# vrettasm/VGPA

Measured on AMD Instinct MI355X. Metric: fwd+bwd sweeps/sec (free-energy+grad eval), Lorenz96 D=40 N=1000, higher is better.
Workload: dtype f64; 1 GPU; Lorenz96 D=40, RK4, Np=1001 (BASELINE configs[2]); batch_per_gpu=512, kernels=mfma

## Files before the change

### vgpa_amd/csrc/energy.hip

```cpp
#include "vgpa_internal.h"
#include "dispatch.h"
#include "energy_small.h"
#include "chol_wave.h"

namespace vgpa {
namespace {

constexpr int NT = 256;

__global__ void __launch_bounds__(NT) k_energy_1d(EnergyArgs a) {
  const int t = blockIdx.x * NT + threadIdx.x;
  const int prob = blockIdx.y;
  if (t >= a.Np) return;
  const size_t o = (size_t)prob * a.Np + t;
  const double la = a.A[(size_t)prob * a.strideA + t], ob = a.b[(size_t)prob * a.strideB + t], m = a.m[o], s = a.S[o];
  Energy1d r;
  const double th = a.theta_v ? a.theta_v[(size_t)prob * kMaxTheta] : a.theta[0];
  const double sg = a.sigma1_v ? a.sigma1_v[prob] : a.sigma1;
  if (a.model == VGPA_MODEL_OU) energy_1d<VGPA_MODEL_OU>(th, sg, la, ob, m, s, r);
  else energy_1d<VGPA_MODEL_DW>(th, sg, la, ob, m, s, r);
  if (a.hyp_only) { a.hyp[o] = r.hyp; return; }
  a.e_t[o] = r.e_t;
  a.Ef[o] = r.ef;
  if (a.Edf) a.Edf[o] = r.edf;
  a.dEm[o] = r.dm;
  a.dEs[o] = r.ds;
  if (a.hyp) a.hyp[o] = r.hyp;
}

__global__ void __launch_bounds__(64) k_energy_l63(EnergyArgs a) {
  const int t = blockIdx.x * 64 + threadIdx.x;
  const int prob = blockIdx.y;
  if (t >= a.Np) return;
  const size_t o = (size_t)prob * a.Np + t;
  const double* At = a.A + (size_t)prob * a.strideA + (size_t)t * 9;
  const double* bt = a.b + (size_t)prob * a.strideB + (size_t)t * 3;
  const double* mt = a.m + o * 3;
  const double* St = a.S + o * 9;
  double Av[9], bv[3], mv[3], Sv[9], isg[3];
  const double* th = a.theta_v ? a.theta_v + (size_t)prob * kMaxTheta : a.theta;
  const double* isgp = a.isg + (size_t)prob * a.isg_stride;
#pragma unroll
  for (int e = 0; e < 9; e++) { Av[e] = At[e]; Sv[e] = St[e]; }
#pragma unroll
  for (int i = 0; i < 3; i++) { bv[i] = bt[i]; mv[i] = mt[i]; isg[i] = isgp[i]; }
  EnergyL63 r;
  if (a.hyp) energy_l63<true>(th, isg, Av, bv, mv, Sv, r); else energy_l63<false>(th, isg, Av, bv, mv, Sv, r);
  if (a.hyp_only) {
    double* hp = a.hyp + o * 6;
#pragma unroll
    for (int i = 0; i < 6; i++) hp[i] = r.hyp[i];
    return;
  }
  a.e_t[o] = r.e_t;
  double* dm = a.dEm + o * 3;
  dm[0] = r.dm[0]; dm[1] = r.dm[1]; dm[2] = r.dm[2];
  double* ds = a.dEs + o * 9;
  ds[0] = r.ds[0]; ds[1] = r.ds[1]; ds[2] = r.ds[2];
  ds[3] = r.ds[1]; ds[4] = r.ds[3]; ds[5] = r.ds[4];
  ds[6] = r.ds[2]; ds[7] = r.ds[4]; ds[8] = r.ds[5];
  double* ef = a.Ef + o * 3;
  ef[0] = r.ef[0]; ef[1] = r.ef[1]; ef[2] = r.ef[2];
  if (a.hyp) {
    double* hp = a.hyp + o * 6;
#pragma unroll
    for (int i = 0; i < 6; i++) hp[i] = r.hyp[i];
  }
  if (a.Edf) {
    double* e = a.Edf + o * 9;
    const double vS = th[0], vR = th[1], vB = th[2];
    e[0] = -vS; e[1] = vS; e[2] = 0.0;
    e[3] = vR - mv[2]; e[4] = -1.0; e[5] = -mv[0];
    e[6] = mv[1]; e[7] = mv[0]; e[8] = -vB;
  }
}

__device__ __forceinline__ int wrap(int i, int n) { return i < 0 ? i + n : (i >= n ? i - n : i); }

__device__ __forceinline__ void wave_sync() {
  __builtin_amdgcn_fence(__ATOMIC_RELEASE, "wavefront");
  __builtin_amdgcn_wave_barrier();
  __builtin_amdgcn_fence(__ATOMIC_ACQUIRE, "wavefront");
}

__device__ __forceinline__ double lane_value(double v, int j) {
  const int lo = __builtin_amdgcn_readlane(__double2loint(v), j);
  const int hi = __builtin_amdgcn_readlane(__double2hiint(v), j);
  return __hiloint2double(hi, lo);
}

using cholw::chol_panel_pivots;
using cholw::rsqrt_pos;

__device__ __forceinline__ double wave_sum(double v) {
#pragma unroll
  for (int o = 32; o > 0; o >>= 1) v += __shfl_xor(v, o, 64);
  return v;
}

template <int NB>
struct WaveGemmGeo {
  static constexpr int NQ = NB / 4, REM = NB % 4, G = REM ? 4 / REM : 0;
  static constexpr int NLEFT = REM ? (NB + G - 1) / G : 0;
  static constexpr int NU = NB * NQ + NLEFT;
};

template <int NB, int MODE, int TRI = 0>
__device__ __forceinline__ void wave_gemm(const double* __restrict__ Aop, const double* __restrict__ Bm, int LD,
                                          double (&acc)[WaveGemmGeo<NB>::NU], const double* __restrict__ bscale = nullptr) {
  using g = WaveGemmGeo<NB>;
  const int l = threadIdx.x & 63, r4 = l >> 4, c4 = l & 3, b = (l >> 2) & 3;
  constexpr int rem = g::REM ? g::REM : 1;
#pragma unroll
  for (int u = 0; u < g::NU; u++) acc[u] = 0.0;
  const double* pa = Aop + r4 * LD + c4;
  const double* pb = Bm + r4 * LD;
  const int colq = l & 15;
  const int coll = 4 * (4 * g::NQ + b % rem) + c4;
  const int ileft = b / rem;
#pragma unroll
  for (int kk = 0; kk < NB; kk++) {
    const double bs = bscale ? bscale[4 * kk + r4] : 1.0;
    double bq[g::NQ > 0 ? g::NQ : 1];
#pragma unroll
    for (int q = 0; q < g::NQ; q++)
      if (kk >= 4 * q) bq[q] = bscale ? bs * pb[kk * 4 * LD + 16 * q + colq] : pb[kk * 4 * LD + 16 * q + colq];
    double bl = 0.0;
    if (g::NLEFT > 0 && kk >= 4 * g::NQ) bl = bscale ? bs * pb[kk * 4 * LD + coll] : pb[kk * 4 * LD + coll];
#pragma unroll
    for (int I = 0; I < NB; I++) {
      if (MODE == 1 && kk < I) continue;
      bool any = false;
#pragma unroll
      for (int q = 0; q < g::NQ; q++) any = any || (kk >= 4 * q && !(TRI == 1 && 4 * q + 3 < I) && !(TRI == 2 && 4 * q > I));
      if (!any) continue;
      const double af = pa[kk * 4 * LD + 4 * I];
#pragma unroll
      for (int q = 0; q < g::NQ; q++)
        if (kk >= 4 * q && !(TRI == 1 && 4 * q + 3 < I) && !(TRI == 2 && 4 * q > I)) acc[q * NB + I] = __builtin_amdgcn_mfma_f64_4x4x4f64(af, bq[q], acc[q * NB + I], 0, 0, 0);
    }
    if (g::NLEFT > 0 && kk >= 4 * g::NQ) {
#pragma unroll
      for (int v = 0; v < g::NLEFT; v++) {
        if (MODE == 1 && kk < v * g::G) continue;
        if (TRI == 2 && v * g::G + g::G - 1 < 4 * g::NQ) continue;
        int ib = v * g::G + ileft;
        ib = ib < NB ? ib : NB - 1;
        const double af = pa[kk * 4 * LD + 4 * ib];
        acc[NB * g::NQ + v] = __builtin_amdgcn_mfma_f64_4x4x4f64(af, bl, acc[NB * g::NQ + v], 0, 0, 0);
      }
    }
  }
}

template <int NB>
__device__ __forceinline__ void wave_gemm_elem(int u, int& row, int& col, bool& ok) {
  using g = WaveGemmGeo<NB>;
  const int l = threadIdx.x & 63, r4 = l >> 4, c4 = l & 3, b = (l >> 2) & 3;
  constexpr int rem = g::REM ? g::REM : 1;
  int Ib, Jb;
  if (u < NB * g::NQ) {
    const int q = u / NB;
    Ib = u - q * NB; Jb = 4 * q + b; ok = true;
  } else {
    const int v = u - NB * g::NQ;
    Ib = v * g::G + b / rem; Jb = 4 * g::NQ + b % rem;
    ok = (b < g::G * g::REM) && (Ib < NB);
  }
  row = 4 * Ib + r4; col = 4 * Jb + c4;
}

struct L96Lds {
  double *Lm, *Gm, *mv, *bv, *am, *sg, *vv, *dl, *qq, *rd;
};

__host__ __device__ inline int l96_dp(int D) { return 4 * ((D + 3) / 4); }
__host__ __device__ inline int l96_ld(int D) { return l96_dp(D) + 1; }
__host__ __device__ inline size_t l96_lds_doubles(int D) {
  return (size_t)2 * l96_dp(D) * l96_ld(D) + 7 * (size_t)l96_dp(D) + (2 * D + 1) + 8 + 4 * (size_t)l96_dp(D);
}

template <int NB>
__global__ void __launch_bounds__(64) k_energy_l96(EnergyArgs a) {
  extern __shared__ __attribute__((aligned(16))) double smem[];
  const int D = a.D, M = 2 * D + 1;
  constexpr int Dp = 4 * NB, LD = Dp + 1;
  const int l = threadIdx.x;
  const long long wid = blockIdx.x;
  const int prob = (int)(wid / a.Np), t = (int)(wid - (long long)prob * a.Np);
  const size_t o = (size_t)prob * a.Np + t;
  L96Lds S;
  S.Lm = smem; S.Gm = S.Lm + Dp * LD; S.mv = S.Gm + Dp * LD; S.bv = S.mv + Dp; S.am = S.bv + Dp; S.sg = S.am + Dp;
  S.dl = S.sg + Dp; S.qq = S.dl + Dp; S.rd = S.qq + Dp; S.vv = S.rd + Dp;
  const double* At = a.A + (size_t)prob * a.strideA + (size_t)t * D * D;
  const double* St = a.S + o * D * D;
  const double theta = a.theta_v ? lds_const(a.theta_v, prob * kMaxTheta) : a.theta[0];
  const double kappa = 1.05 * D, c = D + kappa;
  const bool act = l < D;
  const bool pad = l < Dp;
  const int li = pad ? l : Dp - 1;

  for (int e = l; e < Dp * LD; e += 64) { S.Lm[e] = 0.0; S.Gm[e] = 0.0; }
  if (pad) { S.mv[l] = 0.0; S.bv[l] = 0.0; S.sg[l] = 0.0; S.am[l] = 0.0; S.dl[l] = 0.0; S.qq[l] = 0.0; S.rd[l] = 1.0; }
  wave_sync();
  {
    constexpr int EPL = (Dp * Dp + 63) / 64;
    const int DD = D * D;
    const unsigned magic = ((1u << 20) + (unsigned)D - 1u) / (unsigned)D;
#pragma unroll
    for (int q0 = 0; q0 < EPL; q0 += 9) {
      double sv[9], av[9];
#pragma unroll
      for (int u = 0; u < 9; u++) {
        const int e = l + 64 * (q0 + u);
        const bool in = (q0 + u < EPL) && (e < DD);
        sv[u] = in ? St[e] : 0.0;
        av[u] = in ? At[e] : 0.0;
      }
#pragma unroll
      for (int u = 0; u < 9; u++) {
        const int e = l + 64 * (q0 + u);
        if ((q0 + u < EPL) && (e < DD)) {
          const int r = (int)(((unsigned)e * magic) >> 20), cc = e - r * D;
          S.Lm[r * LD + cc] = c * sv[u];
          S.Gm[cc * LD + r] = av[u];
        }
      }
    }
  }
  if (l >= D && pad) S.Lm[l * LD + l] = 1.0;
  if (act) { S.mv[l] = a.m[o * D + l]; S.bv[l] = a.b[(size_t)prob * a.strideB + (size_t)t * D + l]; S.sg[l] = a.isg[(size_t)prob * a.isg_stride + l]; }
  wave_sync();

  const int r4 = l >> 4, c4 = l & 3, b = (l >> 2) & 3;
  bool bad = false;
  double myrd = 1.0;
  const double* lrow_b = S.Lm + (4 * b + c4) * LD + r4;
  double* lout_b = S.Lm + (4 * b + r4) * LD + c4;
#pragma unroll
  for (int p = 0; p < NB; p++) {
    const int j0 = 4 * p;
    if (p > 0) {
      const double* brow = S.Lm + (j0 + c4) * LD + r4;
#pragma unroll
      for (int u = 0; p + 4 * u < NB; u++) {
        const bool full = p + 4 * u + 3 < NB;
        const bool rowok = full || (p + 4 * u + b < NB);
        const double* arow = full ? lrow_b + 4 * (p + 4 * u) * LD
                                  : S.Lm + (4 * (rowok ? p + 4 * u + b : NB - 1) + c4) * LD + r4;
        double uacc = 0.0;
#pragma unroll
        for (int kk = 0; kk < p; kk++) uacc = __builtin_amdgcn_mfma_f64_4x4x4f64(arow[4 * kk], brow[4 * kk], uacc, 0, 0, 0);
        if (rowok) lout_b[4 * (p + 4 * u) * LD + j0] -= uacc;
      }
      wave_sync();
    }
    chol_panel_pivots<LD>(S.Lm, myrd, j0, l, li, pad);
    wave_sync();
  }
  if (pad) S.rd[l] = myrd;
  wave_sync();
  bad = __any(!(myrd > 0.0 && myrd < __builtin_inf()));
  if (bad) {
    if (l == 0) atomicOr(a.status + prob, 1);
    return;
  }

  double* xdiag = S.vv + (2 * D + 1) + 7;
  if (l < NB) {
    const double* tb = S.Lm + (4 * l) * LD + 4 * l;
    const double x00 = S.rd[4 * l], x11 = S.rd[4 * l + 1], x22 = S.rd[4 * l + 2], x33 = S.rd[4 * l + 3];
    const double t10 = tb[LD], t20 = tb[2 * LD], t21 = tb[2 * LD + 1], t30 = tb[3 * LD], t31 = tb[3 * LD + 1], t32 = tb[3 * LD + 2];
    const double x10 = -(t10 * x00) * x11;
    const double x21 = -(t21 * x11) * x22;
    const double x32 = -(t32 * x22) * x33;
    const double x20 = -(t20 * x00 + t21 * x10) * x22;
    const double x31 = -(t31 * x11 + t32 * x21) * x33;
    const double x30 = -(t30 * x00 + t31 * x10 + t32 * x20) * x33;
    double* xo = xdiag + 16 * l;
    xo[0] = x00; xo[1] = 0.0; xo[2] = 0.0; xo[3] = 0.0;
    xo[4] = x10; xo[5] = x11; xo[6] = 0.0; xo[7] = 0.0;
    xo[8] = x20; xo[9] = x21; xo[10] = x22; xo[11] = 0.0;
    xo[12] = x30; xo[13] = x31; xo[14] = x32; xo[15] = x33;
  }
  {
    double s = 0.0;
#pragma unroll
    for (int k = 0; k < Dp; k++) s = __builtin_fma(S.Gm[k * LD + li], S.mv[k], s);
    if (act) { S.am[l] = s; if (a.Am) a.Am[o * D + l] = s; }
    double acc[WaveGemmGeo<NB>::NU];
    wave_gemm<NB, 0>(S.Gm, S.Lm, LD, acc);
    wave_sync();
#pragma unroll
    for (int u = 0; u < WaveGemmGeo<NB>::NU; u++) {
      int row, col; bool ok;
      wave_gemm_elem<NB>(u, row, col, ok);
      if (ok) S.Gm[row * LD + col] = acc[u];
    }
  }
  wave_sync();

  double vplus = 0.0, vminus = 0.0, v0 = 0.0, r0sq = 0.0;
  const bool hyper = a.hyp != nullptr;
  {
    auto col_of = [&](int q) { return q == 0 ? 0 : (q <= D ? q - 1 : q - 1 - D); };
    auto sgn_of = [&](int q) { return q == 0 ? 0.0 : (q <= D ? 1.0 : -1.0); };
    auto chi = [&](int q, int i) { return S.mv[i] + sgn_of(q) * S.Lm[i * LD + col_of(q)]; };
    const int jc = act ? l : 0;
    const int pP = 1 + jc, pM = 1 + D + jc;
    const int pPm = pP - 1, pPp = pP + 1;
    const int pMm = pM - 1, pMp = wrap(pM + 1, M);
    double am2 = chi(pPm, D - 2), am1 = chi(pPm, D - 1), a0 = chi(pP, 0), a1 = chi(pP, 1);
    double bm2 = chi(pMm, D - 2), bm1 = chi(pMm, D - 1), b0 = chi(pM, 0), b1 = chi(pM, 1);
    const double* lcol = S.Lm + jc;
    const double* gcol = S.Gm + jc;
#pragma unroll
    for (int i = 0; i < Dp; i++) {
      if (i >= D) break;
      const double gi = gcol[i * LD], ami = S.am[i], bvi = S.bv[i], sgi = S.sg[i];
      const double ra = ((a1 - am2) * am1 - a0 + theta) + (ami + gi) - bvi;
      const double rb = ((b1 - bm2) * bm1 - b0 + theta) + (ami - gi) - bvi;
      vplus = __builtin_fma(sgi, ra * ra, vplus);
      vminus = __builtin_fma(sgi, rb * rb, vminus);
      if (hyper && act) S.Gm[i * LD + jc] = ra * ra + rb * rb;
      am2 = am1; am1 = a0; a0 = a1;
      bm2 = bm1; bm1 = b0; b0 = b1;
      const int in = i + 2;
      if (in < D) {
        const double mi = S.mv[in], li2 = lcol[in * LD];
        a1 = mi + li2; b1 = mi - li2;
      } else {
        a1 = chi(pPp, in - D); b1 = chi(pMp, in - D);
      }
    }
    if (act) {
      const int i = l;
      const double xm2 = (i >= 2) ? S.mv[i - 2] : chi(M - 1, D - 2 + i);
      const double xm1 = (i >= 1) ? S.mv[i - 1] : chi(M - 1, D - 1);
      const double x1 = (i + 1 < D) ? S.mv[i + 1] : chi(1, 0);
      const double r0 = ((x1 - xm2) * xm1 - S.mv[i] + theta) + S.am[i] - S.bv[i];
      r0sq = r0 * r0;
      v0 = S.sg[i] * r0sq;
    }
    v0 = wave_sum(v0);
  }
  const double w0 = kappa / c, w1 = 1.0 / (2.0 * c);
  if (hyper) {
    wave_sync();
    if (act) {
      double sm = 0.0;
      for (int j = 0; j < D; j++) sm += S.Gm[l * LD + j];
      const int i = l, ip1 = wrap(i + 1, D), im1 = wrap(i - 1, D), im2 = wrap(i - 2, D);
      const double efi = (St[ip1 * D + im1] - St[im2 * D + im1]) + (S.mv[ip1] - S.mv[im2]) * S.mv[im1] - S.mv[i] + theta;
      double* hp = a.hyp + o * 2 * D;
      hp[i] = efi + S.am[i] - S.bv[i];
      hp[D + i] = w0 * r0sq + w1 * sm;
    }
  }
  const double e_part = act ? (vplus + vminus) : 0.0;
  const double e_t = 0.5 * (w0 * v0 + w1 * wave_sum(e_part));
  if (act) {
    S.dl[l] = w1 * (vplus - vminus);
    S.qq[l] = 0.5 * c * (w1 * (vplus + vminus)) - e_t;
  }
  if (l == 0) a.e_t[o] = e_t;
  wave_sync();

  const double* l4_a = S.Lm + c4 * LD + r4;
  const double* xd_a = xdiag + 4 * c4 + r4;
  const double* xd_d = xdiag + 4 * r4 + c4;
#pragma unroll
  for (int I = 0; I < NB; I++) {
    const double* arow = l4_a + 4 * I * LD;
    const double xd = xd_a[16 * I];
    const double xdd = xd_d[16 * I];
#pragma unroll
    for (int u = 0; 4 * u < NB; u++) {
      const int Jb = 4 * u + b;
      const bool colok = (4 * u + 3 < NB) || (Jb < NB);
      double* xcol = S.Gm + r4 * LD + 4 * (colok ? Jb : NB - 1) + c4;
      double xo = 0.0;
      if (4 * u <= I) {
        double tacc = 0.0;
#pragma unroll
        for (int K = 4 * u; K < I; K++) tacc = __builtin_amdgcn_mfma_f64_4x4x4f64(arow[4 * K], xcol[4 * K * LD], tacc, 0, 0, 0);
        const double prod = __builtin_amdgcn_mfma_f64_4x4x4f64(xd, tacc, 0.0, 0, 0, 0);
        xo = (Jb < I) ? -prod : ((Jb == I) ? xdd : 0.0);
      }
      if (colok) xcol[4 * I * LD] = xo;
    }
    wave_sync();
  }

  {
    double s = 0.0;
    for (int k = 0; k < Dp; k++) s = __builtin_fma(S.Gm[k * LD + li], S.dl[k], s);
    if (act) a.dEm[o * D + l] = 0.5 * c * s;
  }
  double* ds = a.dEs + o * D * D;
  {
    double acc[WaveGemmGeo<NB>::NU];
    wave_gemm<NB, 1>(S.Gm, S.Gm, LD, acc, S.qq);
#pragma unroll
    for (int u = 0; u < WaveGemmGeo<NB>::NU; u++) {
      int row, col; bool ok;
      wave_gemm_elem<NB>(u, row, col, ok);
      if (ok && row < D && col < D && (row <= col || !a.ds_upper)) ds[row * D + col] = 0.5 * c * acc[u];
    }
  }

  if (act) {
    const int i = l, ip1 = wrap(i + 1, D), im1 = wrap(i - 1, D), im2 = wrap(i - 2, D);
    const double cxx = St[ip1 * D + im1] - St[im2 * D + im1];
    a.Ef[o * D + i] = cxx + (S.mv[ip1] - S.mv[im2]) * S.mv[im1] - S.mv[i] + theta;
  }
  if (a.Edf) {
    double* ed = a.Edf + o * D * D;
    for (int e = l; e < D * D; e += 64) {
      const int k = e / D, j = e - k * D;
      const int kp1 = wrap(k + 1, D), km1 = wrap(k - 1, D), km2 = wrap(k - 2, D);
      double v = 0.0;
      if (j == k) v = -1.0;
      if (j == kp1) v = S.mv[km1];
      if (j == km2) v = -S.mv[km1];
      if (j == km1) v = S.mv[kp1] - S.mv[km2];
      ed[e] = v;
    }
  }
}

__host__ __device__ inline bool l96r_compact(int D) { return (D + 3) / 4 == 10; }
__host__ __device__ inline size_t l96r_lds_doubles(int D) {
  const size_t dp = l96_dp(D);
  if (l96r_compact(D)) return dp * l96_ld(D) + 5 * dp;
  return dp * l96_ld(D) + 6 * dp + 9 * dp;
}
template <int R>
__device__ __forceinline__ double row_ror_blocks(double v) {
  typedef int i2_t __attribute__((ext_vector_type(2)));
  i2_t x = __builtin_bit_cast(i2_t, v), y;
  y[0] = __builtin_amdgcn_mov_dpp(x[0], 0x120 + 4 * R, 0xf, 0xf, false);
  y[1] = __builtin_amdgcn_mov_dpp(x[1], 0x120 + 4 * R, 0xf, 0xf, false);
  return __builtin_bit_cast(double, y);
}

struct TriRowTab { unsigned char r[2080]; };
constexpr TriRowTab make_tri_row_tab() {
  TriRowTab t{};
  int e = 0;
  for (int r = 0; r < 64; r++)
    for (int c = 0; c <= r; c++) t.r[e++] = (unsigned char)r;
  return t;
}
__device__ __constant__ TriRowTab kTriRow = make_tri_row_tab();

template <int NB, bool TG = false>
__global__ void __launch_bounds__(64) __attribute__((amdgpu_waves_per_eu(NB <= 10 ? 3 : 2, NB <= 10 ? 3 : 2))) k_energy_l96_r(EnergyArgs a) {
  extern __shared__ __attribute__((aligned(16))) double smem[];
  const int D = a.D, M = 2 * D + 1;
  constexpr int Dp = 4 * NB, LD = Dp + 1, NUU = (NB + 3) / 4;
  const int l = threadIdx.x;
  const long long wid = blockIdx.x;
  const int prob = (int)(wid / a.Np);
  const int t = (int)(wid - (long long)prob * a.Np);
  const size_t o = (size_t)prob * a.Np + t;
  L96Lds S;
  constexpr bool CMP = (NB == 10);
  S.Lm = smem; S.Gm = nullptr; S.mv = S.Lm + Dp * LD; S.bv = S.mv + Dp; S.am = S.bv + Dp; S.sg = nullptr;
  S.dl = S.am + Dp; S.qq = S.dl + Dp; S.rd = CMP ? nullptr : S.qq + Dp; S.vv = CMP ? nullptr : S.rd + Dp;
  double* pv = S.vv;
  double* pw = CMP ? nullptr : pv + 4 * Dp;
  double* gb2 = CMP ? nullptr : pw + 4 * Dp;
  double* xdiag = pv;
  auto cg2 = [&](int j) -> double* { return S.Lm + j * LD + Dp; };
  auto cps = [&](int minus, int j) -> double* { return S.Lm + (4 + 2 * minus + (j >= 20 ? 1 : 0)) * LD + (j >= 20 ? j : 20 + j); };
  auto cxd = [&](int I, int r, int c) -> double* { return S.Lm + ((I < 6 ? 0 : 4) + r) * LD + 4 * (I < 6 ? I + 4 : I - 1) + c; };
  const double* At = a.A + (size_t)prob * a.strideA + (size_t)t * D * D;
  const bool spk = a.s_packed != 0;
  const int PK = tri_off(D);
  const double* St = a.S + o * (spk ? PK : D * D);
  const double theta = a.theta_v ? lds_const(a.theta_v, prob * kMaxTheta) : a.theta[0];
  const double kappa = 1.05 * D, c = D + kappa;
  const bool act = l < D;
  const bool pad = l < Dp;
  const int li = pad ? l : Dp - 1;
  const int r4 = l >> 4, c4 = l & 3, b = (l >> 2) & 3;

  constexpr int NUE = 0;
  double af[NUU][NB];
  const int klim = (D - r4 + 3) >> 2;
  auto load_af = [&](int u) {
    const int row = 16 * u + (l & 15);
    const double* ap = At + row * D + r4;
    const int kl = row < D ? klim : 0;
#pragma unroll
    for (int K = 0; K < NB; K++) af[u][K] = (K < kl) ? ap[4 * K] : 0.0;
  };

  double sxa = 0.0, sxb = 0.0, v_m = 0.0, v_b = 0.0, v_sg = 0.0;
  double nsxa = 0.0, nsxb = 0.0;
  const int f_ip1 = wrap(l + 1, D), f_im1 = wrap(l - 1, D), f_im2 = wrap(l - 2, D);
  if (act) v_sg = a.isg[(size_t)prob * a.isg_stride + l];
  auto load_vectors = [&]() {
    if (act) {
      sxa = St[f_ip1 * D + f_im1];
      sxb = St[f_im2 * D + f_im1];
      v_m = a.m[o * D + l];
      v_b = a.b[(size_t)prob * a.strideB + (size_t)t * D + l];
    }
  };
  constexpr int EPK = (Dp * (Dp + 1) / 2 + 63) / 64;
  double sv[EPK];
  int rr[EPK];
  auto request = [&](int tn) {
    const size_t on = (size_t)prob * a.Np + tn;
    const double* Sn = a.S + on * PK;
#pragma unroll
    for (int q = 0; q < EPK; q++) {
      const int e = l + 64 * q;
      sv[q] = e < PK ? Sn[e] : 0.0;
      rr[q] = kTriRow.r[e < PK ? e : 0];
    }
    if (act) {
      nsxa = Sn[tri_idx(f_ip1, f_im1)];
      nsxb = Sn[tri_idx(f_im2, f_im1)];
      v_m = a.m[on * D + l];
      v_b = a.b[(size_t)prob * a.strideB + (size_t)tn * D + l];
    }
  };
  if (spk) request(t);

  if (spk) {
    if (D != Dp) {
      for (int e = l; e < Dp * LD; e += 64) S.Lm[e] = 0.0;
      wave_sync();
    }
    sxa = nsxa; sxb = nsxb;
#pragma unroll
    for (int q = 0; q < EPK; q++) {
      const int e = l + 64 * q;
      if (e < PK) {
        const int r = rr[q];
        S.Lm[r * LD + (e - tri_off(r))] = c * sv[q];
      }
    }
  } else if (D == Dp) {
    constexpr int RCH = Dp <= 44 ? Dp : 32;
    const double* sp = St + li;
#pragma unroll
    for (int q0 = 0; q0 < Dp; q0 += RCH) {
      double sv[RCH];
#pragma unroll
      for (int u = 0; u < RCH; u++) sv[u] = (q0 + u < Dp) ? sp[(q0 + u) * Dp] : 0.0;
      if (q0 == 0) load_vectors();
      if (pad) {
#pragma unroll
        for (int u = 0; u < RCH; u++)
          if (q0 + u < Dp) S.Lm[(q0 + u) * LD + l] = c * sv[u];
      }
    }
  } else {
    load_vectors();
    for (int e = l; e < Dp * LD; e += 64) S.Lm[e] = 0.0;
    wave_sync();
    constexpr int EPL = (Dp * Dp + 63) / 64;
    constexpr int CH = (NB <= 11) ? EPL : 13;
    const int DD = D * D;
    const unsigned magic = ((1u << 20) + (unsigned)D - 1u) / (unsigned)D;
#pragma unroll
    for (int q0 = 0; q0 < EPL; q0 += CH) {
      double sv[CH];
#pragma unroll
      for (int u = 0; u < CH; u++) {
        const int e = l + 64 * (q0 + u);
        const bool in = (q0 + u < EPL) && (e < DD);
        sv[u] = in ? St[e] : 0.0;
      }
#pragma unroll
      for (int u = 0; u < CH; u++) {
        const int e = l + 64 * (q0 + u);
        if ((q0 + u < EPL) && (e < DD)) {
          const int r = (int)(((unsigned)e * magic) >> 20), cc = e - r * D;
          S.Lm[r * LD + cc] = c * sv[u];
        }
      }
    }
  }
  if (l >= D && pad) S.Lm[l * LD + l] = 1.0;
  if (pad) { S.mv[l] = v_m; S.bv[l] = v_b; S.am[l] = 0.0; }
  wave_sync();

  bool bad = false;
  double myrd = 1.0;
  const double* lrow_b = S.Lm + (4 * b + c4) * LD + r4;
  double* lout_b = S.Lm + (4 * b + r4) * LD + c4;
#pragma unroll
  for (int p = 0; p < NB; p++) {
    const int j0 = 4 * p;
    if (p > 0) {
      const double* brow = S.Lm + (j0 + c4) * LD + r4;
#pragma unroll
      for (int u = 0; p + 4 * u < NB; u++) {
        const bool full = p + 4 * u + 3 < NB;
        const bool rowok = full || (p + 4 * u + b < NB);
        const double* arow = full ? lrow_b + 4 * (p + 4 * u) * LD
                                  : S.Lm + (4 * (rowok ? p + 4 * u + b : NB - 1) + c4) * LD + r4;
        double uacc = 0.0;
#pragma unroll
        for (int kk = 0; kk < p; kk++) uacc = __builtin_amdgcn_mfma_f64_4x4x4f64(arow[4 * kk], brow[4 * kk], uacc, 0, 0, 0);
        if (rowok) lout_b[4 * (p + 4 * u) * LD + j0] -= uacc;
      }
      wave_sync();
    }
    chol_panel_pivots<LD>(S.Lm, myrd, j0, l, li, pad);
    wave_sync();
  }
  if (!CMP && pad) S.rd[l] = myrd;
  wave_sync();
  bad = __any(!(myrd > 0.0 && myrd < __builtin_inf()));
  if (bad) {
    if (l == 0) atomicOr(a.status + prob, 1);
    return;
  }
#pragma unroll
  for (int u = NUE; u < NUU; u++) load_af(u);

  double amr[NUU], gacc[NUU][NB];
#pragma unroll
  for (int u = 0; u < NUU; u++) {
    amr[u] = 0.0;
#pragma unroll
    for (int J = 0; J < NB; J++) gacc[u][J] = 0.0;
  }
#pragma unroll
  for (int pass = 0; pass < (NUE < NUU ? 2 : 1); pass++) {
    const int u0 = pass == 0 ? 0 : NUE, u1 = pass == 0 ? NUE : NUU;
#pragma unroll
    for (int K = 0; K < NB; K++) {
      const double mk = S.mv[4 * K + r4];
#pragma unroll
      for (int u = u0; u < u1; u++) amr[u] = __builtin_amdgcn_mfma_f64_4x4x4f64(af[u][K], mk, amr[u], 0, 0, 0);
      const double* lk = S.Lm + (4 * K + r4) * LD + c4;
#pragma unroll
      for (int J = 0; J <= K; J++) {
        const double lf = lk[4 * J];
#pragma unroll
        for (int u = u0; u < u1; u++) gacc[u][J] = __builtin_amdgcn_mfma_f64_4x4x4f64(af[u][K], lf, gacc[u][J], 0, 0, 0);
      }
    }
  }
#pragma unroll
  for (int u = 0; u < NUU; u++) {
    const int i = 16 * u + 4 * b + r4;
    if (c4 == 0 && i < D) { S.am[i] = amr[u]; if (!TG && a.Am) a.Am[o * D + i] = amr[u]; }
  }
  if constexpr (TG) wave_sync();

  if constexpr (!TG) {
#pragma unroll
  for (int u = 0; u < NUU; u++) {
    if (u == 0 || (16 * u <= Dp - 1 && 16 * u + 15 >= Dp - 4)) {
      const int i = 16 * u + 4 * b + r4;
      if constexpr (CMP) {
        if (i == D - 1) {
#pragma unroll
          for (int J = 0; J < NB; J++) *cg2(4 * J + c4) = gacc[u][J];
        }
      }
      double* gdst = (i == 0) ? S.dl : ((i == 1) ? S.qq : ((i == D - 1 && !CMP) ? gb2 : nullptr));
      if (gdst) {
#pragma unroll
        for (int J = 0; J < NB; J++) gdst[4 * J + c4] = gacc[u][J];
      }
    }
  }
  }
  double tg_edge = 0.0;
  if constexpr (TG) {
    const double w0 = kappa / c, w1 = 1.0 / (2.0 * c);
    auto col_of = [&](int q) { return q == 0 ? 0 : (q <= D ? q - 1 : q - 1 - D); };
    auto sgn_of = [&](int q) { return q == 0 ? 0.0 : (q <= D ? 1.0 : -1.0); };
    auto chi = [&](int q, int i) { return S.mv[i] + sgn_of(q) * S.Lm[i * LD + col_of(q)]; };
    const int jc = act ? l : 0;
    const int pP = 1 + jc, pM = 1 + D + jc;
    const int pPm = pP - 1, pPp = pP + 1;
    const int pMm = pM - 1, pMp = wrap(pM + 1, M);
    const double P0 = chi(pPm, D - 2), P1 = chi(pPm, D - 1), P2 = chi(pP, 0), P3 = chi(pP, 1), P4 = chi(pP, 2);
    const double N0 = chi(pMm, D - 2), N1 = chi(pMm, D - 1), N2 = chi(pM, 0), N3 = chi(pM, 1), N4 = chi(pM, 2);
    const double Q0 = chi(pP, D - 3), Q1 = chi(pP, D - 2), Q2 = chi(pP, D - 1), Q3 = chi(pPp, 0);
    const double R0 = chi(pM, D - 3), R1 = chi(pM, D - 2), R2 = chi(pM, D - 1), R3 = chi(pMp, 0);
    double bsum = 0.0;
    {
      const double lin = S.am[0] - S.bv[0];
      bsum += lane_value(v_sg, 0) * ((((P3 - P0) * P1 - P2 + theta) + lin) + (((N3 - N0) * N1 - N2 + theta) + lin));
    }
    {
      const double lin = S.am[1] - S.bv[1];
      bsum += lane_value(v_sg, 1) * ((((P4 - P1) * P2 - P3 + theta) + lin) + (((N4 - N1) * N2 - N3 + theta) + lin));
    }
    {
      const double lin = S.am[D - 1] - S.bv[D - 1];
      bsum += lane_value(v_sg, D - 1) * ((((Q3 - Q0) * Q1 - Q2 + theta) + lin) + (((R3 - R0) * R1 - R2 + theta) + lin));
    }
    double part = 0.0;
    if (act) {
      const int i = l;
      const double xm2 = (i >= 2) ? S.mv[i - 2] : chi(M - 1, D - 2 + i);
      const double xm1 = (i >= 1) ? S.mv[i - 1] : chi(M - 1, D - 1);
      const double x1 = (i + 1 < D) ? S.mv[i + 1] : chi(1, 0);
      const double r0 = ((x1 - xm2) * xm1 - S.mv[i] + theta) + S.am[i] - S.bv[i];
      part += w1 * bsum + w0 * (v_sg * r0);
    }
    tg_edge = part;
  }
  double vp[NB], vm[NB];
  double tgi = 0.0;
#pragma unroll
  for (int J = 0; J < NB; J++) { vp[J] = 0.0; vm[J] = 0.0; }
  {
#pragma clang fp contract(fast)
#pragma unroll
  for (int u = 0; u < NUU; u++) {
    const int i = 16 * u + 4 * b + r4;
    const bool ok = (i >= 2) && (i <= D - 2);
    const int ir = ok ? i : 2;
    const double mm2 = S.mv[ir - 2], mm1 = S.mv[ir - 1], m0 = S.mv[ir], m1 = S.mv[ir + 1];
    const double sgr = __shfl(v_sg, ir, 64);
    const double bvi = S.bv[ir], sgi = ok ? sgr : 0.0, ami = amr[u];
    const double dm = m1 - mm2;
    const double base = dm * mm1 - m0 + theta + ami - bvi;
    const double* lp = S.Lm + (ir - 2) * LD + c4;
#pragma unroll
    for (int J = 0; J < NB; J++) {
      const double e2 = lp[4 * J], e1 = lp[LD + 4 * J], e0 = lp[2 * LD + 4 * J], ep = lp[3 * LD + 4 * J];
      const double gi = gacc[u][J];
      const double dl = ep - e2;
      const double ev = base + dl * e1;
      const double od = dm * e1 + (dl * mm1 + (gi - e0));
      vp[J] = vp[J] + sgi * (ev * ev + od * od);
      vm[J] = vm[J] + sgi * (ev * od);
      if constexpr (TG) tgi = tgi + ((4 * J + c4 < D) ? sgi : 0.0) * ev;
      if (J == NB / 2 - 1 || J == NB - 1) __builtin_amdgcn_sched_barrier(0);
    }
  }
  }
  if constexpr (TG) {
    const double part = wave_sum(tg_edge + 2.0 * (1.0 / (2.0 * c)) * tgi);
    if (l == 0) a.tg[o] = part;
    return;
  }
  {
    double rp[NB], rm[NB];
#pragma unroll
    for (int J = 0; J < NB; J++) {
      rp[J] = __builtin_amdgcn_mfma_f64_4x4x4f64(1.0, vp[J], 0.0, 0, 0, 0);
      rm[J] = __builtin_amdgcn_mfma_f64_4x4x4f64(1.0, vm[J], 0.0, 0, 0, 0);
    }
    if constexpr (CMP) {
#pragma unroll
      for (int J = 0; J < NB; J++) {
        const double p1 = rp[J] + row_ror_blocks<1>(rp[J]), m1 = rm[J] + row_ror_blocks<1>(rm[J]);
        rp[J] = p1 + row_ror_blocks<2>(p1);
        rm[J] = m1 + row_ror_blocks<2>(m1);
      }
      wave_sync();
      if (r4 == 0 && b == 0) {
#pragma unroll
        for (int J = 0; J < NB; J++) {
          *cps(0, 4 * J + c4) = rp[J];
          *cps(1, 4 * J + c4) = rm[J];
        }
      }
    } else
    if (r4 == 0) {
#pragma unroll
      for (int J = 0; J < NB; J++) {
        pv[b * Dp + 4 * J + c4] = rp[J];
        pw[b * Dp + 4 * J + c4] = rm[J];
      }
    }
  }
  wave_sync();

  double vplus = 0.0, vminus = 0.0, v0 = 0.0;
  {
    auto col_of = [&](int q) { return q == 0 ? 0 : (q <= D ? q - 1 : q - 1 - D); };
    auto sgn_of = [&](int q) { return q == 0 ? 0.0 : (q <= D ? 1.0 : -1.0); };
    auto chi = [&](int q, int i) { return S.mv[i] + sgn_of(q) * S.Lm[i * LD + col_of(q)]; };
    const int jc = act ? l : 0;
    {
      double s1, s2;
      if constexpr (CMP) { s1 = *cps(0, jc); s2 = *cps(1, jc); }
      else {
        s1 = (pv[jc] + pv[Dp + jc]) + (pv[2 * Dp + jc] + pv[3 * Dp + jc]);
        s2 = (pw[jc] + pw[Dp + jc]) + (pw[2 * Dp + jc] + pw[3 * Dp + jc]);
      }
      vplus = s1 + 2.0 * s2;
      vminus = s1 - 2.0 * s2;
    }
    const int pP = 1 + jc, pM = 1 + D + jc;
    const int pPm = pP - 1, pPp = pP + 1;
    const int pMm = pM - 1, pMp = wrap(pM + 1, M);
    {
      const double P0 = chi(pPm, D - 2), P1 = chi(pPm, D - 1), P2 = chi(pP, 0), P3 = chi(pP, 1), P4 = chi(pP, 2);
      const double N0 = chi(pMm, D - 2), N1 = chi(pMm, D - 1), N2 = chi(pM, 0), N3 = chi(pM, 1), N4 = chi(pM, 2);
      const double Q0 = chi(pP, D - 3), Q1 = chi(pP, D - 2), Q2 = chi(pP, D - 1), Q3 = chi(pPp, 0);
      const double R0 = chi(pM, D - 3), R1 = chi(pM, D - 2), R2 = chi(pM, D - 1), R3 = chi(pMp, 0);
      const double g0 = S.dl[jc], g1 = S.qq[jc], g2 = CMP ? *cg2(jc) : gb2[jc];
      {
        const double ami = S.am[0], bvi = S.bv[0], sgi = lane_value(v_sg, 0);
        const double ra = ((P3 - P0) * P1 - P2 + theta) + (ami + g0) - bvi;
        const double rb = ((N3 - N0) * N1 - N2 + theta) + (ami - g0) - bvi;
        vplus = __builtin_fma(sgi, ra * ra, vplus);
        vminus = __builtin_fma(sgi, rb * rb, vminus);
      }
      {
        const double ami = S.am[1], bvi = S.bv[1], sgi = lane_value(v_sg, 1);
        const double ra = ((P4 - P1) * P2 - P3 + theta) + (ami + g1) - bvi;
        const double rb = ((N4 - N1) * N2 - N3 + theta) + (ami - g1) - bvi;
        vplus = __builtin_fma(sgi, ra * ra, vplus);
        vminus = __builtin_fma(sgi, rb * rb, vminus);
      }
      {
        const double ami = S.am[D - 1], bvi = S.bv[D - 1], sgi = lane_value(v_sg, D - 1);
        const double ra = ((Q3 - Q0) * Q1 - Q2 + theta) + (ami + g2) - bvi;
        const double rb = ((R3 - R0) * R1 - R2 + theta) + (ami - g2) - bvi;
        vplus = __builtin_fma(sgi, ra * ra, vplus);
        vminus = __builtin_fma(sgi, rb * rb, vminus);
      }
    }
    if (act) {
      const int i = l;
      const double xm2 = (i >= 2) ? S.mv[i - 2] : chi(M - 1, D - 2 + i);
      const double xm1 = (i >= 1) ? S.mv[i - 1] : chi(M - 1, D - 1);
      const double x1 = (i + 1 < D) ? S.mv[i + 1] : chi(1, 0);
      const double r0 = ((x1 - xm2) * xm1 - S.mv[i] + theta) + S.am[i] - S.bv[i];
      v0 = v_sg * (r0 * r0);
    }
    v0 = wave_sum(v0);
  }
  const double w0 = kappa / c, w1 = 1.0 / (2.0 * c);
  const double e_part = act ? (vplus + vminus) : 0.0;
  const double e_t = 0.5 * (w0 * v0 + w1 * wave_sum(e_part));
  wave_sync();
  if (pad) {
    S.dl[l] = act ? w1 * (vplus - vminus) : 0.0;
    S.qq[l] = act ? 0.5 * c * (w1 * (vplus + vminus)) - e_t : 0.0;
  }
  if (l == 0) a.e_t[o] = e_t;
  const int l4 = l < NB ? 4 * l : 0;
  const double rd0 = CMP ? __shfl(myrd, l4, 64) : 0.0, rd1 = CMP ? __shfl(myrd, l4 + 1, 64) : 0.0;
  const double rd2 = CMP ? __shfl(myrd, l4 + 2, 64) : 0.0, rd3 = CMP ? __shfl(myrd, l4 + 3, 64) : 0.0;
  if (l < NB) {
    const double* tb = S.Lm + (4 * l) * LD + 4 * l;
    const double x00 = CMP ? rd0 : S.rd[4 * l], x11 = CMP ? rd1 : S.rd[4 * l + 1], x22 = CMP ? rd2 : S.rd[4 * l + 2], x33 = CMP ? rd3 : S.rd[4 * l + 3];
    const double t10 = tb[LD], t20 = tb[2 * LD], t21 = tb[2 * LD + 1], t30 = tb[3 * LD], t31 = tb[3 * LD + 1], t32 = tb[3 * LD + 2];
    const double x10 = -(t10 * x00) * x11;
    const double x21 = -(t21 * x11) * x22;
    const double x32 = -(t32 * x22) * x33;
    const double x20 = -(t20 * x00 + t21 * x10) * x22;
    const double x31 = -(t31 * x11 + t32 * x21) * x33;
    const double x30 = -(t30 * x00 + t31 * x10 + t32 * x20) * x33;
    if constexpr (CMP) {
      double* x0 = cxd(l, 0, 0);
      x0[0] = x00; x0[1] = 0.0; x0[2] = 0.0; x0[3] = 0.0;
      x0[LD] = x10; x0[LD + 1] = x11; x0[LD + 2] = 0.0; x0[LD + 3] = 0.0;
      x0[2 * LD] = x20; x0[2 * LD + 1] = x21; x0[2 * LD + 2] = x22; x0[2 * LD + 3] = 0.0;
      x0[3 * LD] = x30; x0[3 * LD + 1] = x31; x0[3 * LD + 2] = x32; x0[3 * LD + 3] = x33;
    } else {
    double* xo = xdiag + 16 * l;
    xo[0] = x00; xo[1] = 0.0; xo[2] = 0.0; xo[3] = 0.0;
    xo[4] = x10; xo[5] = x11; xo[6] = 0.0; xo[7] = 0.0;
    xo[8] = x20; xo[9] = x21; xo[10] = x22; xo[11] = 0.0;
    xo[12] = x30; xo[13] = x31; xo[14] = x32; xo[15] = x33;
    }
  }
  wave_sync();

  const double* l4_a = S.Lm + c4 * LD + r4;
  const double* xd_a = xdiag + 4 * c4 + r4;
  const double* xd_d = xdiag + 4 * r4 + c4;
#pragma unroll
  for (int I = 0; I < NB; I++) {
    const double* arow = l4_a + 4 * I * LD;
    const double xd = CMP ? *cxd(I, c4, r4) : xd_a[16 * I];
    const double xdd = CMP ? *cxd(I, r4, c4) : xd_d[16 * I];
    double xo[NUU];
#pragma unroll
    for (int u = 0; u < NUU; u++) {
      const int Jb = 4 * u + b;
      const bool colok = (4 * u + 3 < NB) || (Jb < NB);
      const double* xcol = S.Lm + r4 * LD + 4 * (colok ? Jb : NB - 1) + c4;
      xo[u] = 0.0;
      if (4 * u <= I) {
        double tacc = 0.0;
#pragma unroll
        for (int K = 4 * u; K < I; K++) tacc = __builtin_amdgcn_mfma_f64_4x4x4f64(arow[4 * K], xcol[4 * K * LD], tacc, 0, 0, 0);
        const double prod = __builtin_amdgcn_mfma_f64_4x4x4f64(xd, tacc, 0.0, 0, 0, 0);
        xo[u] = (Jb < I) ? -prod : ((Jb == I) ? xdd : 0.0);
      }
    }
#pragma unroll
    for (int u = 0; u < NUU; u++) {
      const int Jb = 4 * u + b;
      const bool colok = (4 * u + 3 < NB) || (Jb < NB);
      if (colok && (!CMP || Jb <= I)) S.Lm[(4 * I + r4) * LD + 4 * Jb + c4] = xo[u];
    }
    wave_sync();
  }

  {
    double s = 0.0;
    if constexpr (CMP) {
      const bool z0 = li < 4, z1 = li < 8;
#pragma unroll
      for (int k = 0; k < 8; k++) s = __builtin_fma((k < 4 ? z0 : z1) ? S.Lm[k * LD + li] : 0.0, S.dl[k], s);
      for (int k = 8; k < Dp; k++) s = __builtin_fma(S.Lm[k * LD + li], S.dl[k], s);
    } else
    for (int k = 0; k < Dp; k++) s = __builtin_fma(S.Lm[k * LD + li], S.dl[k], s);
    if (act) a.dEm[o * D + l] = 0.5 * c * s;
  }
  double* ds = a.dEs + o * D * D;
  {
    double acc[WaveGemmGeo<NB>::NU];
    if (a.ds_packed) {
      using gg = WaveGemmGeo<NB>;
      double* dsp = a.dEs + o * PK;
      wave_gemm<NB, 1, 2>(S.Lm, S.Lm, LD, acc, S.qq);
#pragma unroll
      for (int u = 0; u < gg::NU; u++) {
        if (u < NB * gg::NQ && 4 * (u / NB) > u % NB) continue;
        if (u >= NB * gg::NQ && (u - NB * gg::NQ) * gg::G + gg::G - 1 < 4 * gg::NQ) continue;
        int row, col; bool ok;
        wave_gemm_elem<NB>(u, row, col, ok);
        if (ok && row < D && col <= row) dsp[tri_off(row) + col] = 0.5 * c * acc[u];
      }
    } else if (a.ds_upper) {
      wave_gemm<NB, 1, 1>(S.Lm, S.Lm, LD, acc, S.qq);
#pragma unroll
      for (int u = 0; u < WaveGemmGeo<NB>::NU; u++) {
        if (u < NB * WaveGemmGeo<NB>::NQ && 4 * (u / NB) + 3 < u % NB) continue;
        int row, col; bool ok;
        wave_gemm_elem<NB>(u, row, col, ok);
        if (ok && row < D && col < D && row <= col) ds[row * D + col] = 0.5 * c * acc[u];
      }
    } else {
      wave_gemm<NB, 1>(S.Lm, S.Lm, LD, acc, S.qq);
#pragma unroll
      for (int u = 0; u < WaveGemmGeo<NB>::NU; u++) {
        int row, col; bool ok;
        wave_gemm_elem<NB>(u, row, col, ok);
        if (ok && row < D && col < D) ds[row * D + col] = 0.5 * c * acc[u];
      }
    }
  }

  if (act) {
    const int i = l, ip1 = wrap(i + 1, D), im1 = wrap(i - 1, D), im2 = wrap(i - 2, D);
    const double cxx = sxa - sxb;
    a.Ef[o * D + i] = cxx + (S.mv[ip1] - S.mv[im2]) * S.mv[im1] - S.mv[i] + theta;
  }
  if (a.Edf) {
    double* ed = a.Edf + o * D * D;
    for (int e = l; e < D * D; e += 64) {
      const int k = e / D, j = e - k * D;
      const int kp1 = wrap(k + 1, D), km1 = wrap(k - 1, D), km2 = wrap(k - 2, D);
      double v = 0.0;
      if (j == k) v = -1.0;
      if (j == kp1) v = S.mv[km1];
      if (j == km2) v = -S.mv[km1];
      if (j == km1) v = S.mv[kp1] - S.mv[km2];
      ed[e] = v;
    }
  }
}

__global__ void __launch_bounds__(NT) k_edf_dense(EnergyArgs a) {
  const int D = a.D;
  const int t = blockIdx.x, prob = blockIdx.y;
  const size_t o = (size_t)prob * a.Np + t;
  const double* mv = a.m + o * D;
  double* ed = a.Edf + o * D * D;
  const double* th = a.theta_v ? a.theta_v + (size_t)prob * kMaxTheta : a.theta;
  for (int e = threadIdx.x; e < D * D; e += NT) {
    const int k = e / D, j = e - k * D;
    double v = 0.0;
    if (a.model == VGPA_MODEL_L96) {
      const int kp1 = wrap(k + 1, D), km1 = wrap(k - 1, D), km2 = wrap(k - 2, D);
      if (j == k) v = -1.0;
      if (j == kp1) v = mv[km1];
      if (j == km2) v = -mv[km1];
      if (j == km1) v = mv[kp1] - mv[km2];
    } else if (a.model == VGPA_MODEL_L63) {
      const double vS = th[0], vR = th[1], vB = th[2];
      const double tab[9] = {-vS, vS, 0.0, vR - mv[2], -1.0, -mv[0], mv[1], mv[0], -vB};
      v = tab[e];
    } else if (a.model == VGPA_MODEL_OU) {
      v = -th[0];
    } else {
      v = 4.0 * (th[0] - 3.0 * (mv[0] * mv[0] + a.S[o]));
    }
    ed[e] = v;
  }
}

}
}

namespace vgpa {

hipError_t launch_energy(const EnergyArgs& a, hipStream_t st) {
  if (a.model == VGPA_MODEL_OU || a.model == VGPA_MODEL_DW) {
    dim3 grid((a.Np + NT - 1) / NT, a.batch);
    hipLaunchKernelGGL(k_energy_1d, grid, dim3(NT), 0, st, a);
  } else if (a.model == VGPA_MODEL_L63) {
    dim3 grid((a.Np + 63) / 64, a.batch);
    hipLaunchKernelGGL(k_energy_l63, grid, dim3(64), 0, st, a);
  } else if (a.model == VGPA_MODEL_L96) {
    if (a.D < 4 || a.D > kMaxSmallD) return hipErrorInvalidValue;
    const bool one_matrix = (a.hyp == nullptr);
    if (a.tg && !one_matrix) return hipErrorInvalidValue;
    const size_t lds = (one_matrix ? l96r_lds_doubles(a.D) : l96_lds_doubles(a.D)) * sizeof(double);
    const long long nwaves = (long long)a.Np * a.batch;
    if (nwaves > 0x7fffffffLL) return hipErrorInvalidValue;
    return with_int<1, kMaxSmallD / 4>((a.D + 3) / 4, [&](auto nb) {
      constexpr int NB = decltype(nb)::value;
      auto kern = !one_matrix ? k_energy_l96<NB> : a.tg ? k_energy_l96_r<NB, true> : k_energy_l96_r<NB>;
      return launch_lds(kern, dim3((unsigned)nwaves), dim3(64), lds, st, a);
    });
  } else {
    return hipErrorInvalidValue;
  }
  return hipGetLastError();
}

hipError_t launch_edf(const EnergyArgs& a, hipStream_t st) {
  dim3 grid(a.Np, a.batch);
  hipLaunchKernelGGL(k_edf_dense, grid, dim3(NT), 0, st, a);
  return hipGetLastError();
}

}
```

Baseline: 22770 sweeps/s.

## Use 16x16x4 MFMA tiled SYRK for packed dEs gradient with fused dEm

For NB of 9 or 10 with packed dS output, replaces the 4x4 wave_gemm SYRK with a triangular tiled scheme built on 16x16x4 f64 MFMAs. Partial diagonal blocks and the last block-row fall back to 4x4 MFMAs. The dEm matrix-vector product is folded into the same pass over the columns of the factor. The aim is fewer MFMA issues and LDS reads per element of the gradient, at the cost of more accumulator registers and a more complex, compile-time-specialised code path.

```diff
diff --git a/vgpa_amd/csrc/energy.hip b/vgpa_amd/csrc/energy.hip
--- a/vgpa_amd/csrc/energy.hip
+++ b/vgpa_amd/csrc/energy.hip
@@ -169,6 +169,36 @@
   }
   row = 4 * Ib + r4; col = 4 * Jb + c4;
 }
+
+template <int NB>
+struct TileSyrk {
+  static constexpr bool on = (NB == 9 || NB == 10);
+  static constexpr int MT = (NB + 3) / 4, NTILE = (MT - 1) * MT / 2;
+  static constexpr int LAST0 = 4 * (MT - 1), NLAST = on ? NB - LAST0 : 1;
+  static constexpr int tile(int I, int J) { return I * (I + 1) / 2 + J; }
+  static constexpr int first_k(int I) { return 4 * I; }
+  static constexpr int first_row(int I) { return 4 * first_k(I); }
+  static constexpr int whole_k(int I) { return first_k(I) + 3; }
+  static constexpr int products() {
+    int p = 0;
+    for (int I = 0; I < MT - 1; I++) p += (I + 1) * (NB - whole_k(I));
+    return p;
+  }
+  static constexpr int unit_products() {
+    int p = 0;
+    for (int I = 0; I < MT - 1; I++) p += (I + 1) * (1 + 2 + 3);
+    for (int v = 0; v < NLAST; v++) p += MT * (NB - (LAST0 + v));
+    return p;
+  }
+  struct Order { int k[NB]; };
+  static constexpr Order order() {
+    Order o{};
+    int n = 0;
+    for (int K = NB - 1; K >= 8; K--) o.k[n++] = K;
+    for (int s = 0; s < 4; s++) { o.k[n++] = 7 - s; o.k[n++] = 3 - s; }
+    return o;
+  }
+};
 
 struct L96Lds {
   double *Lm, *Gm, *mv, *bv, *am, *sg, *vv, *dl, *qq, *rd;
@@ -909,7 +939,8 @@
     wave_sync();
   }
 
-  {
+  constexpr bool TILE = TileSyrk<NB>::on;
+  if (!(TILE && a.ds_packed)) {
     double s = 0.0;
     if constexpr (CMP) {
       const bool z0 = li < 4, z1 = li < 8;
@@ -923,7 +954,88 @@
   double* ds = a.dEs + o * D * D;
   {
     double acc[WaveGemmGeo<NB>::NU];
-    if (a.ds_packed) {
+    if (TILE && a.ds_packed) {
+      if constexpr (TILE) {
+        using ts = TileSyrk<NB>;
+        static_assert(ts::MT == 3 && ts::first_row(1) >= 8 && ts::first_row(2) >= 8, "rows 0 .. 7 of the columns >= 16 are not X (compact layout)");
+        static_assert(ts::first_row(ts::MT - 1) < Dp && 4 * (NB - 1) + 3 < Dp, "every fragment row lies inside the matrix");
+        static_assert(ts::products() == (NB == 10 ? 13 : 10) && ts::unit_products() == (NB == 10 ? 27 : 21), "k-steps per tile: NB - 4 I - 3; units: 6 per tile, NB - I2 per row block of the last block-row");
+        typedef double d4_t __attribute__((ext_vector_type(4)));
+        constexpr auto ord = ts::order();
+        const int g = l >> 4, n = l & 15;
+        double* dsp = a.dEs + o * PK;
+        const double* xf[ts::MT];
+#pragma unroll
+        for (int I = 0; I < ts::MT; I++) xf[I] = S.Lm + g * LD + (16 * I + n < Dp ? 16 * I + n : Dp - 1);
+        const double* xa = S.Lm + g * LD + c4;
+        d4_t ct[ts::NTILE];
+        double cl[ts::NLAST][ts::MT], dmp[ts::MT];
+#pragma unroll
+        for (int u = 0; u < ts::NTILE; u++) ct[u] = d4_t{0.0, 0.0, 0.0, 0.0};
+#pragma unroll
+        for (int I = 0; I < ts::MT; I++) {
+          dmp[I] = 0.0;
+#pragma unroll
+          for (int v = 0; v < ts::NLAST; v++) cl[v][I] = 0.0;
+        }
+#pragma unroll
+        for (int s = 0; s < NB; s++) {
+          const int K = ord.k[s];
+          const double qk = S.qq[4 * K + g], dk = S.dl[4 * K + g];
+          double fa[ts::MT], fb[ts::MT];
+#pragma unroll
+          for (int I = 0; I < ts::MT; I++)
+            if (ts::first_k(I) <= K) {
+              fa[I] = xf[I][4 * K * LD];
+              fb[I] = qk * fa[I];
+              dmp[I] = __builtin_fma(fa[I], dk, dmp[I]);
+            }
+#pragma unroll
+          for (int I = 0; I < ts::MT - 1; I++) {
+            if (ts::whole_k(I) <= K) {
+#pragma unroll
+              for (int J = 0; J <= I; J++) ct[ts::tile(I, J)] = __builtin_amdgcn_mfma_f64_16x16x4f64(fa[I], fb[J], ct[ts::tile(I, J)], 0, 0, 0);
+            } else if (ts::first_k(I) <= K) {
+#pragma unroll
+              for (int r = 0; r <= K - ts::first_k(I); r++) {
+                const double ar = xa[4 * K * LD + 4 * (ts::first_k(I) + r)];
+#pragma unroll
+                for (int J = 0; J <= I; J++) ct[ts::tile(I, J)][r] = __builtin_amdgcn_mfma_f64_4x4x4f64(ar, fb[J], ct[ts::tile(I, J)][r], 0, 0, 0);
+              }
+            }
+          }
+#pragma unroll
+          for (int v = 0; v < ts::NLAST; v++)
+            if (ts::LAST0 + v <= K) {
+              const double ar = xa[4 * K * LD + 4 * (ts::LAST0 + v)];
+#pragma unroll
+              for (int u = 0; u < ts::MT; u++) cl[v][u] = __builtin_amdgcn_mfma_f64_4x4x4f64(ar, fb[u], cl[v][u], 0, 0, 0);
+            }
+        }
+#pragma unroll
+        for (int I = 0; I < ts::MT; I++) {
+          const double s = __builtin_amdgcn_mfma_f64_4x4x4f64(1.0, dmp[I], 0.0, 0, 0, 0);
+          const int i = 16 * I + n;
+          if (g == 0 && i < D) a.dEm[o * D + i] = 0.5 * c * s;
+        }
+#pragma unroll
+        for (int I = 0; I < ts::MT - 1; I++)
+#pragma unroll
+          for (int J = 0; J <= I; J++)
+#pragma unroll
+            for (int r = 0; r < 4; r++) {
+              const int row = 16 * I + g + 4 * r, col = 16 * J + n;
+              if (row < D && col <= row) dsp[tri_off(row) + col] = 0.5 * c * ct[ts::tile(I, J)][r];
+            }
+#pragma unroll
+        for (int v = 0; v < ts::NLAST; v++)
+#pragma unroll
+          for (int u = 0; u < ts::MT; u++) {
+            const int row = 4 * (ts::LAST0 + v) + g, col = 16 * u + n;
+            if (row < D && col <= row) dsp[tri_off(row) + col] = 0.5 * c * cl[v][u];
+          }
+      }
+    } else if (!TILE && a.ds_packed) {
       using gg = WaveGemmGeo<NB>;
       double* dsp = a.dEs + o * PK;
       wave_gemm<NB, 1, 2>(S.Lm, S.Lm, LD, acc, S.qq);
```

Result: faster. 23030 sweeps/s (median of 6 runs) (+1.2%).
